# dohyeon-Lee/IsaacgymEnv

Hardware: AMD Instinct MI355X
Metric: env-steps/sec AnymalTerrain 4096 envs/GPU (higher is better)
Workload: dtype f32; 1 GPU; AnymalTerrain VecTask.step, terrainType plane (AnymalTerrain.yaml default), 5 physics substeps/step, obs noise on; num_envs_per_gpu=4096, global_num_envs=4096, parallelism=dp1, solver=TGS (physx.solver_type 1, cfg/config.yaml:31)

## Files before the change

### isaacgymenv_amd/csrc/gs_team.hip

```cpp
#include <type_traits>

#include "gs_internal.h"
#include "gs_topologies.h"
#include "gs_math.h"
#include "gs_pairs.h"
#include "gt_anymal_tail.h"

#ifdef GS_PHASE_PROFILE
__device__ unsigned long long gs_phase_cycles[64];
#define GS_PROF_DECL long long gs_t_ = clock64(); long long gs_acc_[16] = {0};
#define GS_PROF(i) { const long long t_ = clock64(); gs_acc_[i] += t_ - gs_t_; gs_t_ = t_; }
#define GS_PROF_COUNT(i, n) { gs_acc_[i] += (n); }
#define GS_PROF_PARAM , long long &gs_t_, long long *gs_acc_
#define GS_PROF_ARGS , gs_t_, gs_acc_
#define GS_PROF_FLUSH                                                   \
  if ((threadIdx.x & 63) == 0) {                                        \
    long long tot_ = 0;                                                 \
    for (int i_ = 0; i_ < 16; ++i_) {                                   \
      atomicAdd(&gs_phase_cycles[i_], (unsigned long long)gs_acc_[i_]); \
      if (i_ < 8 || i_ == 11) tot_ += gs_acc_[i_];                      \
    }                                                                   \
    atomicAdd(&gs_phase_cycles[16 + (int)min(tot_ / 25000, 15ll)], 1ull); \
    if (tot_ > 250000) {                                                \
      for (int i_ = 0; i_ < 16; ++i_) atomicAdd(&gs_phase_cycles[32 + i_], (unsigned long long)gs_acc_[i_]); \
// ... 160 lines not shown
__device__ __forceinline__ void gather_w(int lc, float wA, float wA2, const float (&wC)[T::T_NCH], float* wb,
                                         float* wc) {
  wb[0] = bcast(wA, 0); wb[1] = bcast(wA2, 0); wb[2] = bcast(wA, 1); wb[3] = bcast(wA2, 1);
  wb[4] = bcast(wA, 2); wb[5] = bcast(wA2, 2);
  wc[0] = wc[1] = wc[2] = 0.f;
#pragma unroll
  for (int c = 0; c < T::T_NCH; ++c) {
    const float c0 = bcast(wC[c], 0), c1 = bcast(wC[c], 1), c2 = bcast(wC[c], 2);
    wc[0] = lc == c ? c0 : wc[0];
    wc[1] = lc == c ? c1 : wc[1];
    wc[2] = lc == c ? c2 : wc[2];
  }
}

__device__ __forceinline__ void contact_block(float u0, float u1, float u2, float di0, float di1, float di2,
                                              float s10, float s20, float s21, float tdi, float mu,
                                              float* lam, float& dl0, float& dl1, float& dl2) {
  const float n0 = fmaxf(fmaf(-u0, di0, lam[0] + tdi), 0.f);
  const float a1 = fmaf(-u1, di1, lam[1]);
  const float a2 = fmaf(-u2, di2, lam[2]);
  dl0 = n0 - lam[0];
  lam[0] = n0;
  const float lim = mu * n0;
  const float n1 = __builtin_amdgcn_fmed3f(fmaf(-s10, dl0, a1), -lim, lim);
  const float b2 = fmaf(-s20, dl0, a2);
  dl1 = n1 - lam[1];
  lam[1] = n1;
  const float n2 = __builtin_amdgcn_fmed3f(fmaf(-s21, dl1, b2), -lim, lim);
  dl2 = n2 - lam[2];
  lam[2] = n2;
}

template <class T>
struct TeamState {
  float p[3], quat[4], vo[3], w[3];
  float q[T::T_CL], qd[T::T_CL];
};

template <class T>
__device__ __forceinline__ void stage_chain_model(const DevModel* __restrict__ M, float* mdl) {
  using C = CM<T>;
  for (int i = threadIdx.x; i < C::NP * T::T_NCH; i += blockDim.x) {
    const int p = i / T::T_NCH, c = i - p * T::T_NCH;
    float v;
    if (p < C::CAND) {
      const int k = p / C::BODY, f = p - k * C::BODY;
      const int b = 1 + c * C::CL + k;
      if (f < 9) v = M->jR[b][f];
      else if (f < 12) v = M->jt[b][f - 9];
      else if (f < 15) v = M->jaxis[b][f - 12];
      else if (f < 16) v = M->mass[b];
      else if (f < 19) v = M->com[b][f - 16];
      else v = M->inertia[b][f - 19];
    } else if (p < C::DOF) {
      const int j = (p - C::CAND) / 4, f = (p - C::CAND) - 4 * j;
      const int cand = T::T_RC + c * C::CC + j;
      v = f < 3 ? M->cpoint[cand][f] : M->cradius[cand];
    } else if (p < C::SHP) {
      const int k = (p - C::DOF) / 3, f = (p - C::DOF) - 3 * k;
      const int d = c * C::CL + k;
      v = f == 0 ? M->effort[d] : (f == 1 ? M->vmax[d] : M->armature[d]);
    } else {
      const int j = (p - C::SHP) / 8, f = (p - C::SHP) - 8 * j;
      const int sh = T::T_RS + c * T::T_SPC + j;
      const int kind = M->shkind[sh];
      const float hl = kind == 1 ? M->shsize[sh][1] : 0.f;
      if (f < 6) {
        const float sg = f < 3 ? -hl : hl;
        const int a = f % 3;
        v = kind == 0 || kind == 1 ? M->sht[sh][a] + sg * M->shR[sh][3 * a + 2] : M->shc[sh][a];
      } else if (f == 6) {
        v = kind == 0 || kind == 1 ? M->shm[sh] : M->shc[sh][3];
      } else {
        v = hl;
      }
    }
    mdl[p * C::LANES + c] = v;
  }
}

template <class T>
struct ShapeTab {
  static constexpr int RS = T::HAS_TEAM ? T::T_RS : 0;
  static constexpr int ROOT = kShC * T::NS;
  static constexpr int POSE = ROOT + 8 * RS;
  static constexpr int SIZE = T::NPK > 0 ? POSE + 15 * T::NS : 1;
};
template <class T>
__device__ __forceinline__ void stage_shape_consts(const DevModel* __restrict__ M, float* sct) {
  if constexpr (T::NPK > 0) {
    using S = ShapeTab<T>;
    for (int i = threadIdx.x; i < S::SIZE; i += blockDim.x) {
      float v = 0.f;
      if (i < S::ROOT) {
        const int sh = i / kShC, f = i - kShC * sh;
        v = f == 0 ? M->shc[sh][3]
                   : (f == 1 ? M->shm[sh] : (f == 2 ? M->shsize[sh][1] : (float)(256 * M->shbody[sh] + M->shlink[sh])));
      } else if (i >= S::POSE) {
        const int sh = (i - S::POSE) / 15, f = (i - S::POSE) - 15 * sh;
        v = f < 9 ? M->shR[sh][f] : (f < 12 ? M->sht[sh][f - 9] : M->shc[sh][f - 12]);
      } else {
        const int sr = (i - S::ROOT) / 8, f = (i - S::ROOT) - 8 * sr;
        const int kind = T::shkind[sr];
        const bool seg = kind == 0 || kind == 1;
        const float hl = kind == 1 ? M->shsize[sr][1] : 0.f;
        if (f < 6) {
          const int a = f % 3;
          const float sg = f < 3 ? -hl : hl;
          v = seg ? M->sht[sr][a] + sg * M->shR[sr][3 * a + 2] : M->shc[sr][a];
        } else {
          v = f == 6 ? (seg ? M->shm[sr] : M->shc[sr][3]) : hl;
        }
      }
      sct[i] = v;
    }
  }
}

template <class T>
__device__ __forceinline__ void team_load(const float* __restrict__ st, int N, int e, int lc, TeamState<T>& s) {
  constexpr int ND = T::ND, CL = T::T_CL;
#pragma unroll
  for (int k = 0; k < 3; ++k) s.p[k] = st[k * N + e];
#pragma unroll
  for (int k = 0; k < 4; ++k) s.quat[k] = st[(3 + k) * N + e];
#pragma unroll
  for (int k = 0; k < 3; ++k) s.vo[k] = st[(7 + k) * N + e];
#pragma unroll
  for (int k = 0; k < 3; ++k) s.w[k] = st[(10 + k) * N + e];
#pragma unroll
  for (int k = 0; k < CL; ++k) {
    s.q[k] = st[(13 + lc * CL + k) * N + e];
    s.qd[k] = st[(13 + ND + lc * CL + k) * N + e];
  }
}
template <class T>
__device__ __forceinline__ void team_store(float* __restrict__ st, int N, int e, int lc, const TeamState<T>& s) {
  constexpr int ND = T::ND, CL = T::T_CL;
  if (lc == 0) {
#pragma unroll
    for (int k = 0; k < 3; ++k) st[k * N + e] = s.p[k];
#pragma unroll
    for (int k = 0; k < 4; ++k) st[(3 + k) * N + e] = s.quat[k];
#pragma unroll
    for (int k = 0; k < 3; ++k) st[(7 + k) * N + e] = s.vo[k];
#pragma unroll
    for (int k = 0; k < 3; ++k) st[(10 + k) * N + e] = s.w[k];
  }
#pragma unroll
  for (int k = 0; k < CL; ++k) {
    st[(13 + lc * CL + k) * N + e] = s.q[k];
    st[(13 + ND + lc * CL + k) * N + e] = s.qd[k];
  }
}

__device__ __forceinline__ void body_inertia(const float* R, const float* X, float m, const float* com,
                                             const float* Il, SpI& I) {
  float c[3];
  mat3vec(R, com, c);
  c[0] += X[0]; c[1] += X[1]; c[2] += X[2];
  float Am[9];
#pragma unroll
  for (int r = 0; r < 3; ++r) {
    Am[3 * r + 0] = R[3 * r] * Il[0] + R[3 * r + 1] * Il[3] + R[3 * r + 2] * Il[4];
    Am[3 * r + 1] = R[3 * r] * Il[3] + R[3 * r + 1] * Il[1] + R[3 * r + 2] * Il[5];
    Am[3 * r + 2] = R[3 * r] * Il[4] + R[3 * r + 1] * Il[5] + R[3 * r + 2] * Il[2];
  }
  const float cc = c[0] * c[0] + c[1] * c[1] + c[2] * c[2];
  I.m = m;
  I.h[0] = m * c[0]; I.h[1] = m * c[1]; I.h[2] = m * c[2];
  I.I[0] = Am[0] * R[0] + Am[1] * R[1] + Am[2] * R[2] + m * (cc - c[0] * c[0]);
  I.I[1] = Am[3] * R[3] + Am[4] * R[4] + Am[5] * R[5] + m * (cc - c[1] * c[1]);
  I.I[2] = Am[6] * R[6] + Am[7] * R[7] + Am[8] * R[8] + m * (cc - c[2] * c[2]);
  I.I[3] = Am[0] * R[3] + Am[1] * R[4] + Am[2] * R[5] - m * c[0] * c[1];
  I.I[4] = Am[0] * R[6] + Am[1] * R[7] + Am[2] * R[8] - m * c[0] * c[2];
// ... 472 lines not shown
          o[(kPoolN + k) * RW] = src[(3 + k) * TPW];
        }
        o[kPoolSep * RW] = src[6 * TPW];
        const int a = __float_as_int(src[7 * TPW]), b = __float_as_int(src[8 * TPW]);
        const float nn[3] = {src[3 * TPW], src[4 * TPW], src[5 * TPW]};
        float t1[3], t2[3];
        gs_terrain::tangents(nn, t1, t2);
#pragma unroll
        for (int k = 0; k < 3; ++k) {
          o[(kPoolT1 + k) * RW] = t1[k];
          o[(kPoolT2 + k) * RW] = t2[k];
        }
        o[kPoolMu * RW] = 0.5f * (mu_g[a * N + e] + mu_g[b * N + e]);
        const int bla = (int)sct[kShC * a + 3], blb = (int)sct[kShC * b + 3];
        o[kPoolBA * RW] = (float)(bla >> 8);
        o[kPoolBB * RW] = (float)(blb >> 8);
        o[kPoolLA * RW] = (float)(bla & 255);
        o[kPoolLB * RW] = (float)(blb & 255);
      }
    }
  }
#ifdef GS_PHASE_PROFILE
  {
    const unsigned long long tm = quad_or64(near);
    const unsigned long long lanes = __ballot(tm != 0ull);
    if ((threadIdx.x & 63) == 0) {
      atomicAdd(&gs_phase_cycles[13], (unsigned long long)(clock64() - np_t0));
      atomicAdd(&gs_phase_cycles[15], (unsigned long long)__popcll(lanes));
      atomicAdd(&gs_phase_cycles[10], (unsigned long long)__popcll(tm));
    }
  }
#endif
  return cnt_team;
  }
}

__device__ __forceinline__ float terrain_candidate(const DevParams& P, const float* p, const float* x, float r,
                                                   float* nrm, float& smu) {
  const float cw[3] = {p[0] + x[0], p[1] + x[1], p[2] + x[2]};
  float dist = P.has_ground ? cw[2] - r : 3.0e38f;
  nrm[0] = 0.f; nrm[1] = 0.f; nrm[2] = 1.f;
  smu = P.ground_mu;
  float st, nt[3];
  if (gs_terrain::sphere_contact(P.terr, cw, r, r + P.contact_offset, st, nt) && st < dist) {
    dist = st;
    nrm[0] = nt[0]; nrm[1] = nt[1]; nrm[2] = nt[2];
    smu = P.terr.mu;
  }
  return dist;
}

template <class T>
__device__ __forceinline__ void joint_pose(const float* cm, int k, float qj, const float* Rp, const float* Xp, float* R,
                                           float* X, float* aw) {
  constexpr int LN = T::T_LANES;
  const float* bp = cm + (k * CM<T>::BODY) * LN;
  float jR[9], jt[3], ax[3];
#pragma unroll
  for (int f = 0; f < 9; ++f) jR[f] = bp[f * LN];
#pragma unroll
  for (int f = 0; f < 3; ++f) { jt[f] = bp[(9 + f) * LN]; ax[f] = bp[(12 + f) * LN]; }
  float RJ[9], t[3];
  mat3mul(Rp, jR, RJ);
  mat3vec(Rp, jt, t);
  X[0] = Xp[0] + t[0]; X[1] = Xp[1] + t[1]; X[2] = Xp[2] + t[2];
  mat3vec(RJ, ax, aw);
  if (T::jkind[1 + k] == 1) {
    float sn, cs;
    sincosf(qj, &sn, &cs);
    const float Cc = 1.f - cs;
    float Rq[9];
    Rq[0] = cs + ax[0] * ax[0] * Cc;         Rq[1] = ax[0] * ax[1] * Cc - ax[2] * sn; Rq[2] = ax[0] * ax[2] * Cc + ax[1] * sn;
    Rq[3] = ax[1] * ax[0] * Cc + ax[2] * sn; Rq[4] = cs + ax[1] * ax[1] * Cc;         Rq[5] = ax[1] * ax[2] * Cc - ax[0] * sn;
    Rq[6] = ax[2] * ax[0] * Cc - ax[1] * sn; Rq[7] = ax[2] * ax[1] * Cc + ax[0] * sn; Rq[8] = cs + ax[2] * ax[2] * Cc;
    mat3mul(RJ, Rq, R);
  } else {
#pragma unroll
    for (int f = 0; f < 9; ++f) R[f] = RJ[f];
    X[0] += aw[0] * qj; X[1] += aw[1] * qj; X[2] += aw[2] * qj;
  }
}

template <class T, bool TERR, bool TGS, int EPW, bool ROWL, bool RES>
__device__ __forceinline__ void substep_team(const DevModel* __restrict__ Min, const float* __restrict__ mdl,
                                             const DevParams& P, TeamState<T>& s, const float* tau,
                                             const float* __restrict__ mu_t, int N, int e, int lc,
                                             float* __restrict__ rows_own, const float* __restrict__ rows_team,
                                             float* __restrict__ cf_soa, bool collect,
                                             float* __restrict__ cf_aos, float* __restrict__ shw_tab,
                                             const float* __restrict__ sct, float* __restrict__ stash GS_PROF_PARAM) {
  constexpr int CL = T::T_CL, CC = T::T_CC, RC = T::T_RC, NCH = T::T_NCH, LN = T::T_LANES;
  static_assert(NCH == LN && LN == 4, "lane teams are DPP quads with one chain per lane");
  static_assert(!ROWL || (!TERR && EPW == 4), "row lanes: the 4-envs-per-wave plane form");
  constexpr int NROW = ROWL ? 1 : 3;
  [[maybe_unused]] const int row_own = ROWL ? team_row_of_copy() : 0;
  using C = CM<T>;
  using RS = RowSlots<T>;
  uintptr_t mp = reinterpret_cast<uintptr_t>(Min);
  asm volatile("" : "+s"(mp));
  const DevModel* __restrict__ M = reinterpret_cast<const DevModel*>(mp);
  const float* cm = mdl + lc;
  const float h = P.h;

  float R0[9];
  {
    const float inv = rsqrtf(s.quat[0] * s.quat[0] + s.quat[1] * s.quat[1] + s.quat[2] * s.quat[2] +
                             s.quat[3] * s.quat[3]);
    const float qn[4] = {s.quat[0] * inv, s.quat[1] * inv, s.quat[2] * inv, s.quat[3] * inv};
    quat_to_mat(qn, R0);
  }
  const float X0[3] = {0.f, 0.f, 0.f};
  float nub[6] = {s.w[0], s.w[1], s.w[2], s.vo[0], s.vo[1], s.vo[2]};
  const float A0[6] = {0.f, 0.f, 0.f, -P.g[0], -P.g[1], -P.g[2]};
  SpI I0;
  body_inertia(R0, X0, M->mass[0], M->com[0], M->inertia[0], I0);
  float F0[6];
  {
    float ia[6], iv[6], x6[6];
    spi_mul(I0, A0, ia);
    spi_mul(I0, nub, iv);
    crf(nub, iv, x6);
#pragma unroll
    for (int k = 0; k < 6; ++k) F0[k] = ia[k] + x6[k];
  }

  struct TerrQ {
    float d[CC], n[CC][3], m[CC];
    float rd[RC > 0 ? RC : 1], rn[RC > 0 ? RC : 1][3], rm[RC > 0 ? RC : 1];
  };
  struct NoTerrQ {};
  [[maybe_unused]] std::conditional_t<TERR, TerrQ, NoTerrQ> tq;
  if constexpr (TERR) {
    constexpr int NQ = CC + 1;
    static_assert(RC <= LN, "one root candidate per lane of the team");
    float qc[NQ][3], qr[NQ];
    bool qv[NQ];
    float Rk[9], Xk[3] = {0.f, 0.f, 0.f};
#pragma unroll
    for (int f = 0; f < 9; ++f) Rk[f] = R0[f];
#pragma unroll
    for (int k = 0; k < CL; ++k) {
      float aw[3];
      joint_pose<T>(cm, k, s.q[k], Rk, Xk, Rk, Xk, aw);
#pragma unroll
      for (int j = 0; j < CC; ++j) {
        if (T::T_ccb[j] == k) {
          const float* cp = cm + (C::CAND + 4 * j) * LN;
          const float pl[3] = {cp[0], cp[LN], cp[2 * LN]};
          float x[3];
          mat3vec(Rk, pl, x);
          x[0] += Xk[0]; x[1] += Xk[1]; x[2] += Xk[2];
#pragma unroll
          for (int f = 0; f < 3; ++f) qc[j][f] = s.p[f] + x[f];
          qr[j] = cp[3 * LN];
          qv[j] = true;
        }
      }
    }
    qv[CC] = lc < RC;
    qr[CC] = 0.f;
    qc[CC][0] = qc[CC][1] = qc[CC][2] = 0.f;
    if (lc < RC) {
      float x[3];
      mat3vec(R0, M->cpoint[lc], x);
#pragma unroll
      for (int f = 0; f < 3; ++f) qc[CC][f] = s.p[f] + x[f];
      qr[CC] = M->cradius[lc];
    }
    constexpr int kQItem = 9;
    static_assert(T::NPK > 0 && kShW * T::NS >= kQItem * (CC * LN + RC), "query list fits the pose table");
    float* ql = shw_tab;
    const int wl = threadIdx.x & 63;
    const unsigned long long below = (1ull << wl) - 1ull;
    int slot[NQ];
    int cnt = 0;
#ifdef GS_PHASE_PROFILE
    const long long tq0 = clock64();
#endif
#pragma unroll
    for (int q = 0; q < NQ; ++q) {
      const bool need = qv[q] && gs_terrain::may_contact(P.terr, qc[q], qr[q], qr[q] + P.contact_offset);
      const unsigned long long bal = __ballot(need);
      slot[q] = need ? cnt + __popcll(bal & below) : -1;
      if (need) {
        float* it = ql + slot[q] * kQItem;
        it[0] = qc[q][0]; it[1] = qc[q][1]; it[2] = qc[q][2]; it[3] = qr[q];
      }
      cnt += __popcll(bal);
    }
    team_sync<EPW>();
#ifdef GS_PHASE_PROFILE
    const long long tq1 = clock64();
#endif
    const unsigned long long live = __ballot(true);
    const int nlive = __popcll(live);
    for (int i = __popcll(live & below); i < cnt; i += nlive) {
      float* it = ql + i * kQItem;
      const float cw[3] = {it[0], it[1], it[2]};
      const float r = it[3];
      float st = 0.f, nt[3] = {0.f, 0.f, 1.f};
      const bool found = gs_terrain::sphere_contact_scan(P.terr, cw, r, r + P.contact_offset, st, nt);
      it[4] = found ? 1.f : 0.f;
      it[5] = st;
      it[6] = nt[0]; it[7] = nt[1]; it[8] = nt[2];
    }
    team_sync<EPW>();
#ifdef GS_PHASE_PROFILE
    if ((threadIdx.x & 63) == 0) {
      const long long tq2 = clock64();
      atomicAdd(&gs_phase_cycles[50], (unsigned long long)(tq1 - tq0));
      atomicAdd(&gs_phase_cycles[51], (unsigned long long)(tq2 - tq1));
      atomicAdd(&gs_phase_cycles[52], (unsigned long long)cnt);
    }
#endif
    float rd = 3.0e38f, rn[3] = {0.f, 0.f, 1.f}, rm = P.ground_mu;
#pragma unroll
    for (int q = 0; q < NQ; ++q) {
      float dist = P.has_ground ? qc[q][2] - qr[q] : 3.0e38f;
      float nrm[3] = {0.f, 0.f, 1.f};
      float smu = P.ground_mu;
      if (slot[q] >= 0) {
        const float* it = ql + slot[q] * kQItem;
        if (it[4] != 0.f && it[5] < dist) {
          dist = it[5];
          nrm[0] = it[6]; nrm[1] = it[7]; nrm[2] = it[8];
          smu = P.terr.mu;
        }
      }
      if (q < CC) {
        tq.d[q] = dist; tq.m[q] = smu;
        tq.n[q][0] = nrm[0]; tq.n[q][1] = nrm[1]; tq.n[q][2] = nrm[2];
      } else {
        rd = dist; rm = smu;
        rn[0] = nrm[0]; rn[1] = nrm[1]; rn[2] = nrm[2];
      }
    }
#pragma unroll
    for (int j = 0; j < RC; ++j) {
      tq.rd[j] = bcast(rd, j);
      tq.rm[j] = bcast(rm, j);
#pragma unroll
      for (int f = 0; f < 3; ++f) tq.rn[j][f] = bcast(rn[f], j);
    }
  }

  float R[CL][9], X[CL][3], S[CL][6], V[CL][6], A[CL][6], Fc[CL][6];
  SpI Ic[CL];
  bool act[CC];
  float sep[CC], cmu[CC];
  float cnrm[TERR ? CC : 1][3];
// ... 279 lines not shown
#pragma unroll
      for (int ri = 0; ri < NROW; ++ri) {
        const int rr = ROWL ? row_own : ri;
        float* row = rows_own + (RS::chain(j) + RS::zs(rr, 0)) * RW;
        auto Z = [&](int sl) -> float& { return row[RS::zs(0, sl) * RW]; };
        float zb[6], zc[CL];
        float cj = 0.f;
#pragma unroll
        for (int b = 0; b < 6; ++b) { zb[b] = Z(RS::zslot(b)); cj += zb[b] * nufb[b]; }
#pragma unroll
        for (int k = 0; k < CL; ++k) { zc[k] = Z(RS::zslot(6 + k)); if (k <= kb) cj += zc[k] * nufc[k]; }
#pragma unroll
        for (int kk = 0; kk < CL; ++kk) {
          const int k = kb - kk;
          if (k >= 0) {
#pragma unroll
            for (int i = 0; i < k; ++i) zc[i] -= Mcc[k][i] * zc[k];
#pragma unroll
            for (int b = 0; b < 6; ++b) zb[b] -= Mcb[k][b] * zc[k];
          }
        }
#pragma unroll
        for (int kk = 0; kk < 6; ++kk) {
          const int k = 5 - kk;
#pragma unroll
          for (int b = 0; b < k; ++b) zb[b] -= Mbb[k][b] * zb[k];
        }
        float d = 0.f, zo[6 + CL];
#pragma unroll
        for (int b = 0; b < 6; ++b) {
          zb[b] *= sDb[b];
          d += zb[b] * zb[b];
          Z(RS::zslot(b)) = zb[b];
          zo[b] = zb[b];
        }
#pragma unroll
        for (int k = 0; k < CL; ++k) {
          const float z = k <= kb ? zc[k] * sDc[k] : 0.f;
          d += z * z;
          Z(RS::zslot(6 + k)) = z;
          zo[6 + k] = z;
        }
        Z(3) = 0.f;
        Z(7) = 0.f;
        Z(11) = 0.f;
        Z(12) = 0.f;
        Z(13) = 0.f;
        Z(14) = 0.f;
        Z(RS::CSLOT) = cj;
        const float di = d > 0.f ? __builtin_amdgcn_rcpf(d) : 0.f;
        rec[(RS::C_DI + rr) * RW] = di;
#pragma unroll
        for (int q = 0; q < 3; ++q) {
          if (ROWL || q == ri) {
#pragma unroll
            for (int f = 0; f < 6 + CL; ++f) zr[q][f] = ROWL ? from_copy(zo[f], q) : zo[f];
            dir[q] = ROWL ? from_copy(di, q) : di;
          }
        }
      }
      float g10 = 0.f, g20 = 0.f, g21 = 0.f;
#pragma unroll
      for (int f = 0; f < 6 + CL; ++f) {
        g10 += zr[1][f] * zr[0][f];
        g20 += zr[2][f] * zr[0][f];
        g21 += zr[2][f] * zr[1][f];
      }
      rec[(RS::C_G + 0) * RW] = g10 * dir[1];
      rec[(RS::C_G + 1) * RW] = g20 * dir[2];
      rec[(RS::C_G + 2) * RW] = g21 * dir[2];
      const float sc = sep[j];
      const float tgt = -sc * inv_h;
      rec[RS::C_TP * RW] = (sc < 0.f ? fminf(tgt, P.max_depen_vel) : tgt) * dir[0];
      rec[RS::C_TV * RW] = (sc < 0.f ? 0.f : tgt) * dir[0];
      rec[RS::C_MU * RW] = cmu[j];
      rec[RS::C_SEP * RW] = sc;
    }
  }
  bool ract[RC > 0 ? RC : 1];
  float rnrm[TERR && RC > 0 ? RC : 1][3];
#pragma unroll
  for (int j = 0; j < RC; ++j) {
    float x[3];
    mat3vec(R0, M->cpoint[j], x);
    const float r = M->cradius[j];
    float dist, rmu_s = P.ground_mu;
    float rdir[3][3];
    if constexpr (TERR) {
      dist = tq.rd[j];
      rmu_s = tq.rm[j];
#pragma unroll
      for (int f = 0; f < 3; ++f) rnrm[j][f] = tq.rn[j][f];
      ract[j] = dist < P.contact_offset;
      rdir[0][0] = rnrm[j][0]; rdir[0][1] = rnrm[j][1]; rdir[0][2] = rnrm[j][2];
      gs_terrain::tangents(rnrm[j], rdir[1], rdir[2]);
    } else {
      dist = s.p[2] + x[2] - r;
      ract[j] = P.has_ground && (dist < P.contact_offset);
    }
    if (ract[j]) {
      float* rec = rows_own + RS::root(j) * RW;
      const float xc[3] = {TERR ? x[0] - r * rdir[0][0] : x[0], TERR ? x[1] - r * rdir[0][1] : x[1],
                           TERR ? x[2] - r * rdir[0][2] : x[2] - r};
      float zr[3][6], dir[3];
#pragma unroll
      for (int rr = 0; rr < 3; ++rr) {
        const int ax3 = (rr == 0) ? 2 : (rr == 1 ? 0 : 1);
        float zb[6], cj = 0.f;
        float xd[3] = {0.f, 0.f, 0.f};
        if constexpr (TERR) cross3(xc, rdir[rr], xd);
#pragma unroll
        for (int b = 0; b < 6; ++b) {
          zb[b] = TERR ? (b < 3 ? xd[b] : rdir[rr][b - 3]) : base_jac(xc, ax3, b);
          cj += zb[b] * nufb[b];
        }
#pragma unroll
        for (int kk = 0; kk < 6; ++kk) {
          const int k = 5 - kk;
#pragma unroll
          for (int b = 0; b < k; ++b) zb[b] -= Mbb[k][b] * zb[k];
        }
        float* row = rec + RS::zs(rr, 0) * RW;
        auto Z = [&](int sl) -> float& { return row[RS::zs(0, sl) * RW]; };
        float d = 0.f;
#pragma unroll
        for (int b = 0; b < 6; ++b) {
          zb[b] *= sDb[b];
          d += zb[b] * zb[b];
          Z(RS::zslot(b)) = zb[b];
        }
#pragma unroll
        for (int k = 0; k < 3; ++k) {
          Z(4 * k + 2) = 0.f;
          Z(4 * k + 3) = 0.f;
        }
        Z(12) = 0.f;
        Z(13) = 0.f;
        Z(14) = 0.f;
        Z(RS::CSLOT) = cj;
#pragma unroll
        for (int f = 0; f < 6; ++f) zr[rr][f] = zb[f];
        dir[rr] = d > 0.f ? __builtin_amdgcn_rcpf(d) : 0.f;
        rec[(RS::R_DI + rr) * RW] = dir[rr];
      }
      float g10 = 0.f, g20 = 0.f, g21 = 0.f;
#pragma unroll
      for (int f = 0; f < 6; ++f) {
        g10 += zr[1][f] * zr[0][f];
        g20 += zr[2][f] * zr[0][f];
        g21 += zr[2][f] * zr[1][f];
      }
      rec[(RS::R_G + 0) * RW] = g10 * dir[1];
      rec[(RS::R_G + 1) * RW] = g20 * dir[2];
      rec[(RS::R_G + 2) * RW] = g21 * dir[2];
      const float sc = dist - P.rest_offset;
      const float tgt = -sc * inv_h;
      rec[RS::R_TP * RW] = (sc < 0.f ? fminf(tgt, P.max_depen_vel) : tgt) * dir[0];
      rec[RS::R_TV * RW] = (sc < 0.f ? 0.f : tgt) * dir[0];
      rec[RS::R_MU * RW] = 0.5f * (mu_t[T::T_rcs[j] * kTeamsPerBlock] + rmu_s);
      rec[RS::R_SEP * RW] = sc;
    }
  }
  if constexpr (T::NPK > 0) {
    for (int p = 0; p < npc; ++p) {
      float* o = pool + RS::PER_POOL * p * RW;
      const int ba = (int)o[kPoolBA * RW], bb = (int)o[kPoolBB * RW];
      const int ca = ba > 0 ? (ba - 1) / CL : -1, ka = ba > 0 ? (ba - 1) - ca * CL : -1;
      const int cb = bb > 0 ? (bb - 1) / CL : -1, kb = bb > 0 ? (bb - 1) - cb * CL : -1;
// ... 531 lines not shown
            for (int c = 1; c < NCH; ++c) {
              l0 = lc == c ? lamc[c][j][0] : l0;
              l1 = lc == c ? lamc[c][j][1] : l1;
              l2 = lc == c ? lamc[c][j][2] : l2;
            }
          }
          if constexpr (TERR) {
            float t1[3], t2[3];
            gs_terrain::tangents(cnrm[j], t1, t2);
            f0 += (l0 * cnrm[j][0] + l1 * t1[0] + l2 * t2[0]) * inv_h;
            f1 += (l0 * cnrm[j][1] + l1 * t1[1] + l2 * t2[1]) * inv_h;
            f2 += (l0 * cnrm[j][2] + l1 * t1[2] + l2 * t2[2]) * inv_h;
          } else {
            f0 += l1 * inv_h;
            f1 += l2 * inv_h;
            f2 += l0 * inv_h;
          }
        }
      }
      if constexpr (T::NPK > 0) {
        for (int p = 0; p < npc; ++p) {
          const float* o = pool + RS::PER_POOL * p * RW;
          const int bk = 1 + lc * CL + k;
          const float sg = ((int)o[kPoolBA * RW] == bk ? inv_h : 0.f) - ((int)o[kPoolBB * RW] == bk ? inv_h : 0.f);
          if (sg != 0.f) {
            const float l0 = o[kPoolLam * RW], l1 = o[(kPoolLam + 1) * RW], l2 = o[(kPoolLam + 2) * RW];
            f0 += sg * (l0 * o[kPoolN * RW] + l1 * o[kPoolT1 * RW] + l2 * o[kPoolT2 * RW]);
            f1 += sg * (l0 * o[(kPoolN + 1) * RW] + l1 * o[(kPoolT1 + 1) * RW] + l2 * o[(kPoolT2 + 1) * RW]);
            f2 += sg * (l0 * o[(kPoolN + 2) * RW] + l1 * o[(kPoolT1 + 2) * RW] + l2 * o[(kPoolT2 + 2) * RW]);
          }
        }
      }
      const int b = 1 + lc * CL + k;
      cf_soa[(3 * b + 0) * N + e] = f0;
      cf_soa[(3 * b + 1) * N + e] = f1;
      cf_soa[(3 * b + 2) * N + e] = f2;
      if (cf_aos) {
        float* o = cf_aos + ((size_t)e * T::NB + b) * 3;
        o[0] = f0; o[1] = f1; o[2] = f2;
      }
    }
    if (lc == 0) {
      float f0 = 0.f, f1 = 0.f, f2 = 0.f;
#pragma unroll
      for (int j = 0; j < RC; ++j) {
        if constexpr (TERR) {
          float t1[3], t2[3];
          gs_terrain::tangents(rnrm[j], t1, t2);
          const float g = ract[j] ? inv_h : 0.f;
          f0 += (lamr[j][0] * rnrm[j][0] + lamr[j][1] * t1[0] + lamr[j][2] * t2[0]) * g;
          f1 += (lamr[j][0] * rnrm[j][1] + lamr[j][1] * t1[1] + lamr[j][2] * t2[1]) * g;
          f2 += (lamr[j][0] * rnrm[j][2] + lamr[j][1] * t1[2] + lamr[j][2] * t2[2]) * g;
        } else {
          f0 += lamr[j][1] * inv_h;
          f1 += lamr[j][2] * inv_h;
          f2 += lamr[j][0] * inv_h;
        }
      }
      if constexpr (T::NPK > 0) {
        for (int p = 0; p < npc; ++p) {
          const float* o = pool + RS::PER_POOL * p * RW;
          const float sg = ((int)o[kPoolBA * RW] == 0 ? inv_h : 0.f) - ((int)o[kPoolBB * RW] == 0 ? inv_h : 0.f);
          if (sg != 0.f) {
            const float l0 = o[kPoolLam * RW], l1 = o[(kPoolLam + 1) * RW], l2 = o[(kPoolLam + 2) * RW];
            f0 += sg * (l0 * o[kPoolN * RW] + l1 * o[kPoolT1 * RW] + l2 * o[kPoolT2 * RW]);
            f1 += sg * (l0 * o[(kPoolN + 1) * RW] + l1 * o[(kPoolT1 + 1) * RW] + l2 * o[(kPoolT2 + 1) * RW]);
            f2 += sg * (l0 * o[(kPoolN + 2) * RW] + l1 * o[(kPoolT1 + 2) * RW] + l2 * o[(kPoolT2 + 2) * RW]);
          }
        }
      }
      cf_soa[0 * N + e] = f0;
      cf_soa[1 * N + e] = f1;
      cf_soa[2 * N + e] = f2;
      if (cf_aos) {
        float* o = cf_aos + (size_t)e * T::NB * 3;
        o[0] = f0; o[1] = f1; o[2] = f2;
      }
    }
  }
  GS_PROF(5)
}

template <class T>
__device__ __forceinline__ void team_com_velocity(const DevModel* __restrict__ M, const TeamState<T>& s, float* v) {
  float R[9], c[3], wc[3];
  quat_to_mat(s.quat, R);
  mat3vec(R, M->root_com, c);
  cross3(s.w, c, wc);
  v[0] = s.vo[0] + wc[0]; v[1] = s.vo[1] + wc[1]; v[2] = s.vo[2] + wc[2];
}

__device__ __forceinline__ int xcd_block(int b, int G) {
  constexpr int kXcd = 8;
  const int per = G / kXcd, rem = G % kXcd, x = b % kXcd, q = b / kXcd;
  return x * per + (x < rem ? x : rem) + q;
}

struct TeamLane {
  int wave, col, lc, e;
  bool on, out;
};
template <class T, int EPW, bool ROWL>
__device__ __forceinline__ TeamLane team_lane(int N) {
  constexpr int LN = T::T_LANES;
  static_assert(WaveForm<EPW>::WAVES == 1 || shw_size<T>() % WaveForm<EPW>::WAVES == 0, "every wave its own slice");
  TeamLane t;
  t.wave = WaveForm<EPW>::kWhole ? 0 : (int)(threadIdx.x / GS_WAVE);
  t.col = team_column<EPW, ROWL>();
  t.lc = threadIdx.x & (LN - 1);
  t.on = WaveForm<EPW>::kWhole || ROWL || (int)(threadIdx.x & (GS_WAVE - 1)) < WaveForm<EPW>::LANES;
  t.out = !ROWL || (int)(threadIdx.x & (GS_WAVE - 1)) < WaveForm<EPW>::LANES;
  t.e = t.on ? (xcd_block(blockIdx.x, gridDim.x) * kTeamBlock + t.col) / LN : N;
  return t;
}

template <class T, bool TERR, bool TGS, int EPW, bool ROWL, bool RES>
__global__ __launch_bounds__(WaveForm<EPW>::THREADS, 1) void k_simulate_team(const DevModel* __restrict__ M, DevParams P,
                                                                 SimBuffers B, const float* __restrict__ tau_aos) {
  constexpr int LN = T::T_LANES, CL = T::T_CL, ND = T::ND;
  __shared__ float mdl[CM<T>::NP * LN];
  __shared__ float rows[RowSlots<T>::TOTAL * RW];
  __shared__ float shw_tab[shw_size<T>()];
  __shared__ float sct[ShapeTab<T>::SIZE];
  __shared__ float mu_tab[T::NS * kTeamsPerBlock];
  __shared__ float stash_tab[team_stash_size<T>() * kTeamBlock];
  stage_chain_model<T>(M, mdl);
  stage_shape_consts<T>(M, sct);
  const TeamLane tl = team_lane<T, EPW, ROWL>(B.N);
  const int lc = tl.lc, e = tl.e, col = tl.col;
  if (tl.on)
    for (int sh = lc; sh < T::NS; sh += LN)
      mu_tab[sh * kTeamsPerBlock + (col >> 2)] = e < B.N ? B.mu[(size_t)sh * B.N + e] : 1.f;
  __syncthreads();
  if (e >= B.N) return;
  const float* mu_t = mu_tab + (col >> 2);
  float* shw_wave = shw_tab + tl.wave * (shw_size<T>() / WaveForm<EPW>::WAVES);
  const int N = B.N;
  TeamState<T> s;
  team_load<T>(B.state, N, e, lc, s);
  float tau[CL];
#pragma unroll
  for (int k = 0; k < CL; ++k) tau[k] = tau_aos ? tau_aos[(size_t)e * ND + lc * CL + k] : 0.f;
  float* own = rows + col;
  const float* team = rows + (col & ~(LN - 1));
  GS_PROF_DECL
  for (int sstep = 0; sstep < P.substeps; ++sstep) {
    const bool last = (sstep == P.substeps - 1) && P.collect && tl.out;
    substep_team<T, TERR, TGS, EPW, ROWL, RES>(M, mdl, P, s, tau, mu_t, N, e, lc, own, team, B.cf, last, nullptr, shw_wave, sct, stash_tab + col GS_PROF_ARGS);
  }
  if (tl.out) team_store<T>(B.state, N, opaque_index(e), opaque_index(lc), s);
  GS_PROF_FLUSH
}

template <class T, bool TERR, bool TGS, int EPW, bool ROWL, bool RES>
__global__ __launch_bounds__(WaveForm<EPW>::THREADS, 1) void k_pd_step_team(const DevModel* __restrict__ M, DevParams P,
                                                                SimBuffers B, PdDev A) {
  constexpr int LN = T::T_LANES, CL = T::T_CL, ND = T::ND, NB = T::NB;
  __shared__ float mdl[CM<T>::NP * LN];
  __shared__ float rows[RowSlots<T>::TOTAL * RW];
  __shared__ float shw_tab[shw_size<T>()];
  __shared__ float sct[ShapeTab<T>::SIZE];
  __shared__ float mu_tab[T::NS * kTeamsPerBlock];
  __shared__ float stash_tab[team_stash_size<T>() * kTeamBlock];
  stage_chain_model<T>(M, mdl);
  stage_shape_consts<T>(M, sct);
  const TeamLane tl = team_lane<T, EPW, ROWL>(B.N);
  const int lc = tl.lc, e = tl.e, col = tl.col;
  if (tl.on)
    for (int sh = lc; sh < T::NS; sh += LN)
      mu_tab[sh * kTeamsPerBlock + (col >> 2)] = e < B.N ? B.mu[(size_t)sh * B.N + e] : 1.f;
  __syncthreads();
  if (e >= B.N) return;
  const float* mu_t = mu_tab + (col >> 2);
  float* shw_wave = shw_tab + tl.wave * (shw_size<T>() / WaveForm<EPW>::WAVES);
  const int N = B.N;
  TeamState<T> s;
  team_load<T>(B.state, N, e, lc, s);
  float tau[CL];
  float* own = rows + col;
  const float* team = rows + (col & ~(LN - 1));
  const int sub = P.substeps;
  const int n_pd = A.decimation * sub;
  const int total = (A.decimation + A.extra) * sub;
  auto dof0 = [&]() { return (size_t)opaque_index(e) * ND + lc * CL; };
  GS_PROF_DECL
  for (int it = 0; it < total; ++it) {
    if (it < n_pd && (it % sub) == 0) {
      const bool first = it == 0;
      const size_t d0 = dof0();
#pragma unroll
      for (int k = 0; k < CL; ++k) {
        const float qj = first ? A.dof_state_in[(d0 + k) * 2 + 0] : s.q[k];
        const float qdj = first ? A.dof_state_in[(d0 + k) * 2 + 1] : s.qd[k];
        const float aj = A.actions[d0 + k];
        tau[k] = clampf(A.kp * (A.scale * aj + A.default_pos[lc * CL + k] - qj) - A.kd * qdj, -A.tlim, A.tlim);
      }
    }
    const bool last = it == total - 1 && P.collect && tl.out;
    GS_PROF(6)
    float* cf_aos = (it == total - 1) ? A.cf_out : nullptr;
    substep_team<T, TERR, TGS, EPW, ROWL, RES>(M, mdl, P, s, tau, mu_t, N, e, lc, own, team, B.cf, last, cf_aos, shw_wave, sct, stash_tab + col GS_PROF_ARGS);
    if (it == n_pd - 1 && A.dof_out && tl.out) {
      const size_t d0 = dof0();
#pragma unroll
      for (int k = 0; k < CL; ++k) {
        A.dof_out[(d0 + k) * 2 + 0] = s.q[k];
        A.dof_out[(d0 + k) * 2 + 1] = s.qd[k];
      }
    }
  }
  if (tl.out) {
    team_store<T>(B.state, N, opaque_index(e), opaque_index(lc), s);
    const size_t d0 = dof0();
#pragma unroll
    for (int k = 0; k < CL; ++k) A.torques_out[d0 + k] = tau[k];
    if (A.actions_copy) {
#pragma unroll
      for (int k = 0; k < CL; ++k) A.actions_copy[d0 + k] = A.actions[d0 + k];
    }
  }
  if (A.root_out && lc == 0 && tl.out) {
    float* o = A.root_out + (size_t)e * 13;
    o[0] = s.p[0]; o[1] = s.p[1]; o[2] = s.p[2];
    o[3] = s.quat[0]; o[4] = s.quat[1]; o[5] = s.quat[2]; o[6] = s.quat[3];
    float v[3];
    team_com_velocity<T>(M, s, v);
    o[7] = v[0]; o[8] = v[1]; o[9] = v[2];
    o[10] = s.w[0]; o[11] = s.w[1]; o[12] = s.w[2];
  }
  if constexpr (!TERR && EPW == 16) if (kTeamsPerBlock == 16 && A.tail_on) {
    __syncthreads();
    const bool reset = lc == 0 && (ND == 12 ? gt_tail::post_a_env<true, false, (ND == 12 ? 12 : 0)>(
                                                  A.tail_p, A.tail_b, gt_anymal_hound{}, e)
                                            : gt_tail::post_a_env<true, false>(A.tail_p, A.tail_b, gt_anymal_hound{}, e));
    const unsigned long long m = __ballot(reset);
    unsigned m16 = 0;
#pragma unroll
    for (int i = 0; i < kTeamsPerBlock; ++i) m16 |= (unsigned)((m >> (LN * i)) & 1ull) << i;
    const int e0 = e - (int)(threadIdx.x / LN);
    const unsigned long long live = __ballot(true);
    if ((int)(threadIdx.x & 63) == __ffsll((long long)live) - 1) {
      uint16_t* slices = reinterpret_cast<uint16_t*>(A.tail_b.reset_masks);
      slices[e0 / kTeamsPerBlock] = (uint16_t)m16;
      if (e0 + kTeamsPerBlock >= N)
        for (int q = e0 / kTeamsPerBlock + 1; q % 4 != 0; ++q) slices[q] = 0;
      gt_tail::publish_count(A.tail_b, (unsigned)__popc(m16), gridDim.x);
    }
  }
  GS_PROF(7)
  GS_PROF_FLUSH
}

}

bool team_fused_tail_available() { return kTeamsPerBlock == 16; }

constexpr int kTeamEpwPlane = 4, kTeamEpwTerr = 16;
static int team_epw(const DevParams& P, bool tail) {
  if (kTeamBlock != GS_WAVE || tail) return 16;
  const int w = P.team_epw > 0 ? P.team_epw : (P.has_terrain ? kTeamEpwTerr : kTeamEpwPlane);
  return w == 8 || w == 4 ? w : 16;
}
constexpr bool kTeamRowLanesPlane = true;
static bool team_row_lanes(const DevParams& P, int epw) {
  if (kTeamBlock != GS_WAVE || epw != 4 || P.has_terrain) return false;
  return P.team_row_lanes >= 0 ? P.team_row_lanes != 0 : kTeamRowLanesPlane;
}
constexpr bool kTeamResidentPlane = true;
static bool team_resident_sweeps(const DevParams& P, int epw) {
  if (!team_row_lanes(P, epw)) return false;
  return P.team_resident >= 0 ? P.team_resident != 0 : kTeamResidentPlane;
}
void team_launch_form(const DevParams& P, int* epw, int* row_lanes) {
  *epw = team_epw(P, false);
  *row_lanes = team_row_lanes(P, *epw) ? 1 : 0;
}
int team_launch_resident(const DevParams& P) { return team_resident_sweeps(P, team_epw(P, false)) ? 1 : 0; }
#define GS_TEAM_LAUNCH_EPW(K, EPW, ...)                                                                      \
  do {                                                                                                       \
    const dim3 g_((unsigned)blocks), b_((unsigned)WaveForm<EPW>::THREADS);                                   \
    if (P.has_terrain && P.tgs) hipLaunchKernelGGL((K<T, true, true, EPW, false, false>), g_, b_, 0, st, __VA_ARGS__);  \
    else if (P.has_terrain) hipLaunchKernelGGL((K<T, true, false, EPW, false, false>), g_, b_, 0, st, __VA_ARGS__); \
    else if (P.tgs) hipLaunchKernelGGL((K<T, false, true, EPW, false, false>), g_, b_, 0, st, __VA_ARGS__);         \
    else hipLaunchKernelGGL((K<T, false, false, EPW, false, false>), g_, b_, 0, st, __VA_ARGS__);                   \
  } while (0)
#define GS_TEAM_LAUNCH_ROWL(K, ...)                                                                          \
  do {                                                                                                       \
    const dim3 g_((unsigned)blocks), b_((unsigned)WaveForm<4>::THREADS);                                     \
    const bool res_ = team_resident_sweeps(P, 4);                                                            \
    if (P.tgs && res_) hipLaunchKernelGGL((K<T, false, true, 4, true, true>), g_, b_, 0, st, __VA_ARGS__);   \
    else if (P.tgs) hipLaunchKernelGGL((K<T, false, true, 4, true, false>), g_, b_, 0, st, __VA_ARGS__);     \
    else if (res_) hipLaunchKernelGGL((K<T, false, false, 4, true, true>), g_, b_, 0, st, __VA_ARGS__);      \
    else hipLaunchKernelGGL((K<T, false, false, 4, true, false>), g_, b_, 0, st, __VA_ARGS__);               \
  } while (0)
#define GS_TEAM_LAUNCH(K, epw, ...)                              \
  do {                                                           \
    if constexpr (kTeamBlock == GS_WAVE) {                       \
      if ((epw) == 8) { GS_TEAM_LAUNCH_EPW(K, 8, __VA_ARGS__); break; }  \
      if ((epw) == 4 && team_row_lanes(P, 4)) { GS_TEAM_LAUNCH_ROWL(K, __VA_ARGS__); break; }  \
      if ((epw) == 4) { GS_TEAM_LAUNCH_EPW(K, 4, __VA_ARGS__); break; }  \
    }                                                            \
    GS_TEAM_LAUNCH_EPW(K, 16, __VA_ARGS__);                      \
  } while (0)

template <class T>
hipError_t launch_sim_team(const DevModel* M, const DevParams& P, const SimBuffers& B, const float* tau,
                           hipStream_t st) {
  if constexpr (T::HAS_TEAM) {
    static_assert(T::NR == T::NB, "the lane team reports contact forces per body (no kept fixed-joint links)");
// ... 40 lines not shown
```

Baseline: 37.39 million env-steps/s.

## Stage root body constants in LDS and hoist per-env global loads before staging

Result: faster. 38.08 million env-steps/s, median of 6 (+1.8%).

```diff
diff --git a/isaacgymenv_amd/csrc/gs_team.hip b/isaacgymenv_amd/csrc/gs_team.hip
--- a/isaacgymenv_amd/csrc/gs_team.hip
+++ b/isaacgymenv_amd/csrc/gs_team.hip
@@ -266,15 +266,29 @@
 template <class T>
 struct ShapeTab {
   static constexpr int RS = T::HAS_TEAM ? T::T_RS : 0;
+  static constexpr int RC = T::HAS_TEAM ? T::T_RC : 0;
   static constexpr int ROOT = kShC * T::NS;
   static constexpr int POSE = ROOT + 8 * RS;
-  static constexpr int SIZE = T::NPK > 0 ? POSE + 15 * T::NS : 1;
+  static constexpr int SHAPES = T::NPK > 0 ? POSE + 15 * T::NS : 0;
+  static constexpr int BODY0 = SHAPES;
+  static constexpr int RCAND = BODY0 + 10;
+  static constexpr int RCOM = RCAND + 4 * RC;
+  static constexpr int SIZE = RCOM + 3;
 };
 template <class T>
 __device__ __forceinline__ void stage_shape_consts(const DevModel* __restrict__ M, float* sct) {
+  using S = ShapeTab<T>;
+  for (int i = S::SHAPES + (int)threadIdx.x; i < S::SIZE; i += blockDim.x) {
+    const int f = i - S::BODY0;
+    float v;
+    if (i < S::RCAND) v = f == 0 ? M->mass[0] : (f < 4 ? M->com[0][f - 1] : M->inertia[0][f - 4]);
+    else if (i < S::RCOM) v = ((i - S::RCAND) & 3) < 3 ? M->cpoint[(i - S::RCAND) >> 2][(i - S::RCAND) & 3]
+                                                       : M->cradius[(i - S::RCAND) >> 2];
+    else v = M->root_com[i - S::RCOM];
+    sct[i] = v;
+  }
   if constexpr (T::NPK > 0) {
-    using S = ShapeTab<T>;
-    for (int i = threadIdx.x; i < S::SIZE; i += blockDim.x) {
+    for (int i = threadIdx.x; i < S::SHAPES; i += blockDim.x) {
       float v = 0.f;
       if (i < S::ROOT) {
         const int sh = i / kShC, f = i - kShC * sh;
@@ -913,7 +927,7 @@
 }
 
 template <class T, bool TERR, bool TGS, int EPW, bool ROWL, bool RES>
-__device__ __forceinline__ void substep_team(const DevModel* __restrict__ Min, const float* __restrict__ mdl,
+__device__ __forceinline__ void substep_team(const DevModel* __restrict__ M, const float* __restrict__ mdl,
                                              const DevParams& P, TeamState<T>& s, const float* tau,
                                              const float* __restrict__ mu_t, int N, int e, int lc,
                                              float* __restrict__ rows_own, const float* __restrict__ rows_team,
@@ -927,9 +941,8 @@
   [[maybe_unused]] const int row_own = ROWL ? team_row_of_copy() : 0;
   using C = CM<T>;
   using RS = RowSlots<T>;
-  uintptr_t mp = reinterpret_cast<uintptr_t>(Min);
-  asm volatile("" : "+s"(mp));
-  const DevModel* __restrict__ M = reinterpret_cast<const DevModel*>(mp);
+  const float* rb0 = sct + ShapeTab<T>::BODY0;
+  [[maybe_unused]] const float* rcand = sct + ShapeTab<T>::RCAND;
   const float* cm = mdl + lc;
   const float h = P.h;
 
@@ -944,7 +957,7 @@
   float nub[6] = {s.w[0], s.w[1], s.w[2], s.vo[0], s.vo[1], s.vo[2]};
   const float A0[6] = {0.f, 0.f, 0.f, -P.g[0], -P.g[1], -P.g[2]};
   SpI I0;
-  body_inertia(R0, X0, M->mass[0], M->com[0], M->inertia[0], I0);
+  body_inertia(R0, X0, rb0[0], rb0 + 1, rb0 + 4, I0);
   float F0[6];
   {
     float ia[6], iv[6], x6[6];
@@ -993,10 +1006,10 @@
     qc[CC][0] = qc[CC][1] = qc[CC][2] = 0.f;
     if (lc < RC) {
       float x[3];
-      mat3vec(R0, M->cpoint[lc], x);
+      mat3vec(R0, rcand + 4 * lc, x);
 #pragma unroll
       for (int f = 0; f < 3; ++f) qc[CC][f] = s.p[f] + x[f];
-      qr[CC] = M->cradius[lc];
+      qr[CC] = rcand[4 * lc + 3];
     }
     constexpr int kQItem = 9;
     static_assert(T::NPK > 0 && kShW * T::NS >= kQItem * (CC * LN + RC), "query list fits the pose table");
@@ -1442,8 +1455,8 @@
 #pragma unroll
   for (int j = 0; j < RC; ++j) {
     float x[3];
-    mat3vec(R0, M->cpoint[j], x);
-    const float r = M->cradius[j];
+    mat3vec(R0, rcand + 4 * j, x);
+    const float r = rcand[4 * j + 3];
     float dist, rmu_s = P.ground_mu;
     float rdir[3][3];
     if constexpr (TERR) {
@@ -2141,10 +2154,10 @@
 }
 
 template <class T>
-__device__ __forceinline__ void team_com_velocity(const DevModel* __restrict__ M, const TeamState<T>& s, float* v) {
+__device__ __forceinline__ void team_com_velocity(const float* __restrict__ sct, const TeamState<T>& s, float* v) {
   float R[9], c[3], wc[3];
   quat_to_mat(s.quat, R);
-  mat3vec(R, M->root_com, c);
+  mat3vec(R, sct + ShapeTab<T>::RCOM, c);
   cross3(s.w, c, wc);
   v[0] = s.vo[0] + wc[0]; v[1] = s.vo[1] + wc[1]; v[2] = s.vo[2] + wc[2];
 }
@@ -2183,23 +2196,25 @@
   __shared__ float sct[ShapeTab<T>::SIZE];
   __shared__ float mu_tab[T::NS * kTeamsPerBlock];
   __shared__ float stash_tab[team_stash_size<T>() * kTeamBlock];
+  const TeamLane tl = team_lane<T, EPW, ROWL>(B.N);
+  const int lc = tl.lc, e = tl.e, col = tl.col;
+  const int N = B.N;
+  TeamState<T> s;
+  float tau[CL];
+  if (e < N) {
+    team_load<T>(B.state, N, e, lc, s);
+#pragma unroll
+    for (int k = 0; k < CL; ++k) tau[k] = tau_aos ? tau_aos[(size_t)e * ND + lc * CL + k] : 0.f;
+  }
   stage_chain_model<T>(M, mdl);
   stage_shape_consts<T>(M, sct);
-  const TeamLane tl = team_lane<T, EPW, ROWL>(B.N);
-  const int lc = tl.lc, e = tl.e, col = tl.col;
   if (tl.on)
     for (int sh = lc; sh < T::NS; sh += LN)
-      mu_tab[sh * kTeamsPerBlock + (col >> 2)] = e < B.N ? B.mu[(size_t)sh * B.N + e] : 1.f;
+      mu_tab[sh * kTeamsPerBlock + (col >> 2)] = e < N ? B.mu[(size_t)sh * N + e] : 1.f;
   __syncthreads();
-  if (e >= B.N) return;
+  if (e >= N) return;
   const float* mu_t = mu_tab + (col >> 2);
   float* shw_wave = shw_tab + tl.wave * (shw_size<T>() / WaveForm<EPW>::WAVES);
-  const int N = B.N;
-  TeamState<T> s;
-  team_load<T>(B.state, N, e, lc, s);
-  float tau[CL];
-#pragma unroll
-  for (int k = 0; k < CL; ++k) tau[k] = tau_aos ? tau_aos[(size_t)e * ND + lc * CL + k] : 0.f;
   float* own = rows + col;
   const float* team = rows + (col & ~(LN - 1));
   GS_PROF_DECL
@@ -2220,39 +2235,59 @@
   __shared__ float shw_tab[shw_size<T>()];
   __shared__ float sct[ShapeTab<T>::SIZE];
   __shared__ float mu_tab[T::NS * kTeamsPerBlock];
-  __shared__ float stash_tab[team_stash_size<T>() * kTeamBlock];
+  constexpr bool kActRegs = !TERR;
+  constexpr int kActSlot = team_stash_size<T>();
+  __shared__ float stash_tab[(team_stash_size<T>() + (kActRegs ? 0 : CL)) * kTeamBlock];
+  __shared__ float dpos_tab[ND];
+  const TeamLane tl = team_lane<T, EPW, ROWL>(B.N);
+  const int lc = tl.lc, e = tl.e, col = tl.col;
+  const int N = B.N;
+  auto dof0 = [&]() { return (size_t)opaque_index(e) * ND + lc * CL; };
+  TeamState<T> s;
+  float q_in[CL], qd_in[CL];
+  [[maybe_unused]] float act[CL];
+  if (e < N) {
+    team_load<T>(B.state, N, e, lc, s);
+    const size_t d0 = dof0();
+#pragma unroll
+    for (int k = 0; k < CL; ++k) {
+      q_in[k] = A.dof_state_in[(d0 + k) * 2 + 0];
+      qd_in[k] = A.dof_state_in[(d0 + k) * 2 + 1];
+      const float aj = A.actions[d0 + k];
+      if constexpr (kActRegs) act[k] = aj;
+      else stash_tab[(kActSlot + k) * kTeamBlock + col] = aj;
+    }
+  }
   stage_chain_model<T>(M, mdl);
   stage_shape_consts<T>(M, sct);
-  const TeamLane tl = team_lane<T, EPW, ROWL>(B.N);
-  const int lc = tl.lc, e = tl.e, col = tl.col;
+  for (int i = threadIdx.x; i < ND; i += blockDim.x) dpos_tab[i] = A.default_pos[i];
   if (tl.on)
     for (int sh = lc; sh < T::NS; sh += LN)
-      mu_tab[sh * kTeamsPerBlock + (col >> 2)] = e < B.N ? B.mu[(size_t)sh * B.N + e] : 1.f;
+      mu_tab[sh * kTeamsPerBlock + (col >> 2)] = e < N ? B.mu[(size_t)sh * N + e] : 1.f;
   __syncthreads();
-  if (e >= B.N) return;
+  if (e >= N) return;
   const float* mu_t = mu_tab + (col >> 2);
   float* shw_wave = shw_tab + tl.wave * (shw_size<T>() / WaveForm<EPW>::WAVES);
-  const int N = B.N;
-  TeamState<T> s;
-  team_load<T>(B.state, N, e, lc, s);
+  auto action = [&](int k) {
+    if constexpr (kActRegs) return act[k];
+    else return stash_tab[(kActSlot + k) * kTeamBlock + col];
+  };
   float tau[CL];
   float* own = rows + col;
   const float* team = rows + (col & ~(LN - 1));
   const int sub = P.substeps;
   const int n_pd = A.decimation * sub;
   const int total = (A.decimation + A.extra) * sub;
-  auto dof0 = [&]() { return (size_t)opaque_index(e) * ND + lc * CL; };
   GS_PROF_DECL
   for (int it = 0; it < total; ++it) {
     if (it < n_pd && (it % sub) == 0) {
       const bool first = it == 0;
-      const size_t d0 = dof0();
 #pragma unroll
       for (int k = 0; k < CL; ++k) {
-        const float qj = first ? A.dof_state_in[(d0 + k) * 2 + 0] : s.q[k];
-        const float qdj = first ? A.dof_state_in[(d0 + k) * 2 + 1] : s.qd[k];
-        const float aj = A.actions[d0 + k];
-        tau[k] = clampf(A.kp * (A.scale * aj + A.default_pos[lc * CL + k] - qj) - A.kd * qdj, -A.tlim, A.tlim);
+        const float qj = first ? q_in[k] : s.q[k];
+        const float qdj = first ? qd_in[k] : s.qd[k];
+        const float aj = action(k);
+        tau[k] = clampf(A.kp * (A.scale * aj + dpos_tab[lc * CL + k] - qj) - A.kd * qdj, -A.tlim, A.tlim);
       }
     }
     const bool last = it == total - 1 && P.collect && tl.out;
@@ -2275,7 +2310,7 @@
     for (int k = 0; k < CL; ++k) A.torques_out[d0 + k] = tau[k];
     if (A.actions_copy) {
 #pragma unroll
-      for (int k = 0; k < CL; ++k) A.actions_copy[d0 + k] = A.actions[d0 + k];
+      for (int k = 0; k < CL; ++k) A.actions_copy[d0 + k] = action(k);
     }
   }
   if (A.root_out && lc == 0 && tl.out) {
@@ -2283,7 +2318,7 @@
     o[0] = s.p[0]; o[1] = s.p[1]; o[2] = s.p[2];
     o[3] = s.quat[0]; o[4] = s.quat[1]; o[5] = s.quat[2]; o[6] = s.quat[3];
     float v[3];
-    team_com_velocity<T>(M, s, v);
+    team_com_velocity<T>(sct, s, v);
     o[7] = v[0]; o[8] = v[1]; o[9] = v[2];
     o[10] = s.w[0]; o[11] = s.w[1]; o[12] = s.w[2];
   }
```
